# vivek87799/lightweight-human-pose-estimation.pytorch

Hardware: AMD Instinct MI355X
Metric: frames/sec end-to-end (net+grouping) at 368px (higher is better)
Workload: dtype f32; 1 GPU; batch=1 per GPU, 368x656 frames, 1 refinement stage(s), fp32 convs / f32+f64 post, resident normalised NCHW input -> key-points + pose entries on host; 3 frame batch(es) in flight per GPU (3 engine stream(s), each step a complete pass); global_batch=1, parallelism=dp1 (frames sharded, no data-path collective), 3 stream(s) per GPU

## Files before the change

lightweight-human-pose-estimation.pytorch_amd/csrc/lwp_internal.h:

```cpp
#pragma once
#include <hip/hip_runtime.h>
#include <stdint.h>
#include <algorithm>
#include <cstdio>
#include <string>
#include <vector>

#include "../../include/lwpose.h"

namespace lwp {

struct ParamSpec {
    std::string key;
    int64_t shape[4];
    int ndim;
    int role;
};
std::vector<ParamSpec> param_table(int nref, int C, int NH, int NP);

enum LayerKind { L_STEM = 0, L_DW = 1, L_GEMM = 2, L_DWPW = 3 };
enum Act { ACT_NONE = 0, ACT_RELU = 1, ACT_ELU = 2 };
enum KClass { KC_STEM = 0, KC_DW = 1, KC_PW = 2, KC_C3 = 3, KC_POST = 4, KC_OTHER = 5, KC_COUNT = 6 };

struct BufRef {
    int buf = -1;
    int coff = 0;
    int ld = 0;
};

struct WBlock {
    std::string conv_key;
    int out_off, in_off, cout, cin;
};

struct Layer {
    int kind = L_GEMM;
    std::string name;
    std::string conv_key;
    std::string bn_key;
    bool has_bias = false;
    int cin = 0, cout = 0, ks = 1, stride = 1, dil = 1, act = ACT_NONE;
    BufRef src, dst, res;
    int out_index = -1;
    int out_index2 = -1, out_split = 0;
    std::vector<WBlock> blocks;
    int64_t macs_per_pixel = 0;
    int fuse = LWP_MARK_NONE;
    size_t w_off = 0, b_off = 0;
    int cin_pad = 0, cout_pad = 0;
    std::string conv2_key, bn2_key;
    int act2 = ACT_NONE;
    size_t w2_off = 0, b2_off = 0;
};

struct BufSpec {
    int level;
    int channels;
    bool has_pad = false;
};

struct Graph {
    int nref, C, NH, NP;
    std::vector<BufSpec> bufs;
    std::vector<Layer> layers;
    size_t blob_floats = 0;
    int cat_buf = -1;
    int cat_channels = 0;
    int dtype = LWP_F32;
};
Graph build_graph(int nref, int C, int NH, int NP, bool fuse_dwpw, int dtype, bool merge_heads = true);

struct TrainPlan {
    std::vector<Layer> layers;
    std::vector<BufSpec> bufs;
    std::vector<int> cats;
    int cpm_conv = -1;
    int cpm_in = -1;
    int cut = -1;
    std::vector<int> dw_copy, nores_copy;
    enum { GRAD_ALWAYS = 0, GRAD_NEVER = 1, GRAD_ON_DEMAND = 2 };
    std::vector<char> grad_mode;
};
TrainPlan build_train_plan(const Graph& g, int scope = LWP_TRAIN_STAGES);
uint16_t f32_to_f16_rne(float f);
uint16_t f32_to_bf16_rne(float f);

struct HostTensor {
    const void* ptr;
    int64_t shape[4];
    int ndim;
};
std::string pack_weights(const Graph& g, const std::vector<std::string>& names,
                         const std::vector<HostTensor>& tensors, std::vector<float>& blob);

struct Tuning {
    int stem_ty = 0, stem_wl = -1, stem_debug = 0;
    int dw_tiled = -1, dw_cc = 0, dw_ph = 0;
    int gemm_wp = -1;
    bool has_c3 = false, has_pw = false; int c3[3] = {0, 0, 0}, pw[3] = {0, 0, 0};
    int dwpw_bm = 0, dwpw_nw = 0, dwpw_debug = 0, dwpwh_debug = 0;
    int dwpw_pipe = -1;
    int dwpw_tiled_wgs = 0;
    int dwpw_tiled = -1;
    int dwpw_pp_grid = 0;
    int dwpw_pp = -1;
    int heads_rm = 0;
    int gemmh_fold = -1;
    int gemmh_persist = -1, gemmh_ar_off = 0, gemmh_ar_force = 0, gemmh_debug = 0;
    bool has_gemmh_ar = false, has_gemmh = false; int gemmh_ar[4] = {0, 0, 0, 0}, gemmh[4] = {0, 0, 0, 0};
    int upsample_tiled = -1;
    int max_frames_per_pass = 0;
    int peak_tile = -1, pair_form = -1;
    int dwpw_lds_pad_kb = 0;
    int host_fetch_dma = -1;
    int ms_tx = 0;
    int ms_vec = -1;
    int ms_fused = -1;
    int heads_f32_lds = -1;
    int post_nchw = -1;
    int heads_f32_max_m = 0;
    int fuse_dwpw = -1, merge_heads = -1, fuse_heads = -1;
    int pre_batch_vec = -1;
    int post_stream = -1, post_generic = -1;
};
Tuning tuning_from_env();
const Tuning& default_tuning();
constexpr int kVariantCap = 64;
#define LWP_VARIANT(p, ...) do { if ((p).variant) snprintf((p).variant, lwp::kVariantCap, __VA_ARGS__); } while (0)

struct StemParams {
    const float* __restrict__ in;
    const float* __restrict__ w;
    const float* __restrict__ bias;
    float* __restrict__ out;
    int N, H, W, Ho, Wo;
    int f16 = 0;
    const float* zeros = nullptr;
    const Tuning* tune = nullptr; char* variant = nullptr;
};
struct DwParams {
    const float* in; int in_ld;
    const float* w;
    const float* bias;
    float* out; int out_ld;
    int N, Hi, Wi, Ho, Wo, C, stride, dil, act;
    const Tuning* tune = nullptr; char* variant = nullptr;
};
struct GemmParams {
    const float* in; int in_ld;
    int f16 = 0;
    const float* w;
    const float* wf = nullptr;
    const float* bias;
    float* out; int out_ld;
    const float* res; int res_ld;
    float* out_nchw;
    float* out_nchw2 = nullptr;
    int out_split = 0;
    const float* zeros;
    int N, H, W, cin_pad, cout, cout_pad, ks, dil, act;
    int debug = 0;
    const Tuning* tune = nullptr; char* variant = nullptr;
    const void* w2 = nullptr; const float* bias2 = nullptr; void* out2 = nullptr; int out2_ld = 0, act2 = 0;
    bool* fused2 = nullptr;
};
struct DwPwParams {
    const float* in; int in_ld;
    int f16 = 0;
    const float* dw_w;
    const float* pw_w;
    const float* pw_b;
    float* out; int out_ld;
    const float* res; int res_ld;
    const float* zeros;
    int N, Hi, Wi, Ho, Wo, C, cout, stride, dil, act_dw, act_pw;
    int debug = 0;
    const Tuning* tune = nullptr; char* variant = nullptr;
};
bool dwpw_supported(int C, int cout);
hipError_t launch_dwpw(const DwPwParams& p, hipStream_t s);
hipError_t try_dwpw_tiled_f32(const DwPwParams& p, hipStream_t s, bool* used);
// ... 386 lines not shown
```

lightweight-human-pose-estimation.pytorch_amd/csrc/net_kernels.hip:

```cpp
#include <cstdio>
#include <cstdlib>

#include <type_traits>
#include "lwp_internal.h"

namespace lwp {

typedef float f32x4 __attribute__((ext_vector_type(4)));
typedef float f32x2 __attribute__((ext_vector_type(2)));
typedef float f32x16 __attribute__((ext_vector_type(16)));

__device__ __forceinline__ float elu_negative(float v) {
    const float p = v * (1.f + v * (0.5f + v * (1.f / 6.f + v * (1.f / 24.f + v * (1.f / 120.f + v * (1.f / 720.f + v * (1.f / 5040.f)))))));
    return v > -0.5f ? p : __expf(v) - 1.0f;
}
__device__ __forceinline__ float apply_act(float v, int act) {
    if (act == ACT_RELU) return fmaxf(v, 0.0f);
    if (act == ACT_ELU) return v > 0.0f ? v : elu_negative(v);
    return v;
}

constexpr int ST_TX = 32;
template <bool BF16, int ST_TY, int PY = 1, int DBG = 0, bool WL = false, bool F16 = false>
__global__ void __launch_bounds__(ST_TY * ST_TX) stem_kernel(StemParams p) {
// ... 635 lines not shown
                acc = __builtin_amdgcn_mfma_f32_32x32x2f32(av[s].z, bv[s].z, acc, 0, 0, 0);
                acc = __builtin_amdgcn_mfma_f32_32x32x2f32(av[s].w, bv[s].w, acc, 0, 0, 0);
            }
        }
        if (nxt < nsteps) {
            store_step();
#pragma unroll
            for (int s = 0; s < BK / 8; ++s) bv[s] = b_nxt[s];
        }
    }

    float resv[16];
    const bool has_res = p.res != nullptr && g == 0 && n < p.cout;
    if (has_res) {
#pragma unroll
        for (int i = 0; i < 16; ++i) {
            const int m = m0 + (i & 3) + 8 * (i >> 2) + 4 * h;
            resv[i] = m < M ? p.res[(int64_t)m * p.res_ld + n] : 0.f;
        }
    }
    if (KS > 1) {
        __syncthreads();
        float* red = smem;
        if (g > 0) {
#pragma unroll
            for (int i = 0; i < 16; ++i) red[(((g - 1) * WN + wn) * 16 + i) * 64 + lane] = acc[i];
        }
        __syncthreads();
        if (g > 0) return;
#pragma unroll 1
        for (int gg = 1; gg < KS; ++gg)
#pragma unroll
            for (int i = 0; i < 16; ++i) acc[i] += red[(((gg - 1) * WN + wn) * 16 + i) * 64 + lane];
    }

    if (n < p.cout) {
        const int HW = p.H * p.W;
#pragma unroll
        for (int i = 0; i < 16; ++i) {
            const int m = m0 + (i & 3) + 8 * (i >> 2) + 4 * h;
            if (m < M) {
                float v = apply_act(acc[i] + bias, p.act);
                if (has_res) v += resv[i];
                p.out[(int64_t)m * p.out_ld + n] = v;
                if (p.out_nchw || p.out_nchw2) {
                    const int img = m / HW, pix = m - img * HW;
                    const int c0 = p.out_split > 0 ? p.out_split : p.cout;
                    if (n < c0) { if (p.out_nchw) p.out_nchw[((int64_t)img * c0 + n) * HW + pix] = v; }
                    else if (p.out_nchw2) p.out_nchw2[((int64_t)img * (p.cout - c0) + (n - c0)) * HW + pix] = v;
                }
            }
        }
    }
}

template <int BN, int KS, int KSZ>
static hipError_t launch_gemm_wp_k(const GemmParams& p, hipStream_t s) {
    const int64_t M = (int64_t)p.N * p.H * p.W;
    if (M >= (1ll << 31) - 64) return hipErrorInvalidValue;
    const int64_t tiles = ((M + 31) / 32) * (p.cout_pad / BN);
    constexpr int NWV = (BN / 32) * KS;
    size_t lds = (size_t)NWV * 32 * LDS_LD * sizeof(float);
    const size_t red = (size_t)(KS - 1) * (BN / 32) * 16 * 64 * sizeof(float);
    if (red > lds) lds = red;
    if (!p.wf) return hipErrorInvalidValue;
    static LdsAttrOnce attr;
    if (lds > 64 * 1024) {
        hipError_t e = attr.ensure((const void*)gemm_wp_kernel<BN, KS, KSZ>, (int)lds);
        if (e != hipSuccess) return e;
    }
    hipLaunchKernelGGL((gemm_wp_kernel<BN, KS, KSZ>), dim3((unsigned)tiles), dim3(NWV * 64), lds, s, p);
    return hipGetLastError();
}
template <int BN, int KS>
static hipError_t launch_gemm_wp_t(const GemmParams& p, hipStream_t s) {
    if (p.ks == 3) return launch_gemm_wp_k<BN, KS, 3>(p, s);
    if (p.ks == 1) return launch_gemm_wp_k<BN, KS, 1>(p, s);
    return hipErrorInvalidValue;
}

#ifndef AR_PF
#define AR_PF 2
#endif
template <int BN, int KS, int KSZ>
__global__ void __launch_bounds__((BN / 32) * KS * 64) gemm_ar_kernel(GemmParams p) {
    constexpr int WN = BN / 32;
    constexpr int GT = WN * 64;
    extern __shared__ __attribute__((aligned(16))) float smem[];
    const int tid = threadIdx.x, lane = tid & 63;
    const int wave = __builtin_amdgcn_readfirstlane(tid >> 6);
    const int g = wave / WN, wn = wave % WN;
    const int r = lane & 31, h = lane >> 5;

    const int M = p.N * p.H * p.W;
    const int ntn = p.cout_pad / BN;
    int bid = blockIdx.x;
    {
        const int nwg = gridDim.x, q = nwg >> 3, rem = nwg & 7, xcd = bid & 7;
        bid = (xcd < rem ? xcd * (q + 1) : rem * (q + 1) + (xcd - rem) * q) + (bid >> 3);
    }
    const int tile_m = bid / ntn, tile_n = bid % ntn;
    const int m0 = tile_m * 32;
    const int n0 = tile_n * BN + wn * 32;
    const int n = n0 + r;
    const float bias = n < p.cout ? p.bias[n] : 0.f;

    const int kpt = p.cin_pad / BK;
    const int nb = g < kpt ? (kpt - g + KS - 1) / KS : 0;
    const int nb_max = (kpt + KS - 1) / KS;
    const int seg = KSZ == 3 ? 32 + 2 * p.dil : 32;
    const int R = KSZ == 3 ? 3 * seg : 32;
    float* Ag = smem + (size_t)g * (nb_max * R + 1) * LDS_LD;
    float* zrow = Ag + (size_t)nb_max * R * LDS_LD;

    const __amdgpu_buffer_rsrc_t arsrc = __builtin_amdgcn_make_buffer_rsrc((void*)p.in, 0, (int)((int64_t)M * p.in_ld * 4), 0x00020000);
    {
        const int t = tid - g * GT;
        const int col = (t & 7) * 4;
        const int total = nb * R;
        for (int base = 0; base < total; base += 8 * (GT / 8)) {
            f32x4 tmp[8];
#pragma unroll
            for (int u = 0; u < 8; ++u) {
                const int ch = base + (t >> 3) + u * (GT / 8);
                const int chc = ch < total ? ch : 0;
                const int j = chc / R, row = chc - j * R;
                int64_t idx;
                if (KSZ == 3) {
                    const int sd = row / seg, rw = row - sd * seg;
                    idx = (int64_t)m0 + (int64_t)(sd - 1) * p.dil * p.W - p.dil + rw;
                } else {
                    idx = (int64_t)m0 + row;
                }
                const bool ok = ch < total && idx >= 0 && idx < M;
                tmp[u] = __builtin_bit_cast(f32x4, __builtin_amdgcn_raw_buffer_load_b128(arsrc, ok ? (unsigned)(((int)idx * p.in_ld + (g + j * KS) * BK + col) * 4) : 0x80000000u, 0, 0));
            }
#pragma unroll
            for (int u = 0; u < 8; ++u) {
                const int ch = base + (t >> 3) + u * (GT / 8);
                if (ch < total) *(f32x4*)(Ag + (size_t)ch * LDS_LD + col) = tmp[u];
            }
        }
        if (t < 9) *(f32x4*)(zrow + 4 * t) = f32x4{0.f, 0.f, 0.f, 0.f};
    }

    const int mrow = m0 + r;
    const bool row_ok = mrow < M;
    const int mm = row_ok ? mrow : 0;
    const int qy = mm / p.W;
    const int x = mm - qy * p.W, y = qy % p.H;
    unsigned valid = 0;
#pragma unroll
    for (int t = 0; t < KSZ * KSZ; ++t) {
        const int yy = y + (KSZ == 3 ? (t / 3 - 1) * p.dil : 0), xx = x + (KSZ == 3 ? (t % 3 - 1) * p.dil : 0);
        if (row_ok && yy >= 0 && yy < p.H && xx >= 0 && xx < p.W) valid |= 1u << t;
    }
    constexpr int taps = KSZ * KSZ;
    const int my_steps = nb * taps;
    const __amdgpu_buffer_rsrc_t wrsrc = __builtin_amdgcn_make_buffer_rsrc((void*)p.wf, 0, 0x7fffffff, 0x00020000);
    const unsigned b_tile = (unsigned)__builtin_amdgcn_readfirstlane(n0 >> 5) * 4096u;
    const unsigned b_step = (unsigned)(p.cout_pad >> 5) * 4096u;
    auto load_b = [&](int i, f32x4* dst) {
        const int j = i / taps, tap = i - j * taps;
        const unsigned soff = (unsigned)(tap * kpt + g + j * KS) * b_step + b_tile;
#pragma unroll
        for (int s = 0; s < BK / 8; ++s) dst[s] = __builtin_bit_cast(f32x4, __builtin_amdgcn_raw_buffer_load_b128(wrsrc, lane * 16 + s * 1024, soff, 0));
    };
    constexpr int PF = AR_PF;
    f32x4 bv[PF][BK / 8];
    if (my_steps > 0) {
#pragma unroll
        for (int u = 0; u < PF - 1; ++u) load_b(u < my_steps ? u : my_steps - 1, bv[u]);
    }
    __syncthreads();

    f32x16 acc = {0.f, 0.f, 0.f, 0.f, 0.f, 0.f, 0.f, 0.f, 0.f, 0.f, 0.f, 0.f, 0.f, 0.f, 0.f, 0.f};
    const float* a_lane = Ag + (size_t)r * LDS_LD + 4 * h;
    const float* z_lane = zrow + 4 * h;
    auto one = [&](int i, auto P_) {
        constexpr int P = decltype(P_)::value;
        const int nxt = i + PF - 1 < my_steps ? i + PF - 1 : my_steps - 1;
        load_b(nxt, bv[(P + PF - 1) % PF]);
        const int j = i / taps, tap = i - j * taps;
        int roff = j * R;
        if (KSZ == 3) roff += (tap / 3) * seg + (tap % 3) * p.dil;
        const float* a = (valid >> tap) & 1u ? a_lane + (size_t)roff * LDS_LD : z_lane;
        f32x4 av[BK / 8];
#pragma unroll
        for (int s = 0; s < BK / 8; ++s) av[s] = *(const f32x4*)(a + 8 * s);
#pragma unroll
        for (int s = 0; s < BK / 8; ++s) {
            acc = __builtin_amdgcn_mfma_f32_32x32x2f32(av[s].x, bv[P][s].x, acc, 0, 0, 0);
            acc = __builtin_amdgcn_mfma_f32_32x32x2f32(av[s].y, bv[P][s].y, acc, 0, 0, 0);
            acc = __builtin_amdgcn_mfma_f32_32x32x2f32(av[s].z, bv[P][s].z, acc, 0, 0, 0);
            acc = __builtin_amdgcn_mfma_f32_32x32x2f32(av[s].w, bv[P][s].w, acc, 0, 0, 0);
        }
    };
    int i = 0;
    for (; i + PF <= my_steps; i += PF) {
        one(i, std::integral_constant<int, 0>{});
        if (PF > 1) one(i + 1, std::integral_constant<int, 1 % PF>{});
        if (PF > 2) one(i + 2, std::integral_constant<int, 2 % PF>{});
        if (PF > 3) one(i + 3, std::integral_constant<int, 3 % PF>{});
    }
    if (i < my_steps) { one(i, std::integral_constant<int, 0>{}); ++i; }
    if (PF > 2 && i < my_steps) { one(i, std::integral_constant<int, 1 % PF>{}); ++i; }
    if (PF > 3 && i < my_steps) { one(i, std::integral_constant<int, 2 % PF>{}); ++i; }

    constexpr int EPG = 16 / KS;
    const int e0 = g * EPG;
    float resv[EPG];
    const bool has_res = p.res != nullptr && n < p.cout;
    if (has_res) {
#pragma unroll
        for (int u = 0; u < EPG; ++u) {
            const int e = e0 + u;
            const int m = m0 + (e & 3) + 8 * (e >> 2) + 4 * h;
            resv[u] = m < M ? p.res[(int64_t)m * p.res_ld + n] : 0.f;
        }
    }
    float outv[EPG];
    if (KS > 1) {
        __syncthreads();
        float* red = smem;
#pragma unroll
        for (int e = 0; e < 16; ++e) red[((g * WN + wn) * 16 + e) * 64 + lane] = acc[e];
        __syncthreads();
#pragma unroll
        for (int u = 0; u < EPG; ++u) {
            float v = red[((0 * WN + wn) * 16 + e0 + u) * 64 + lane];
#pragma unroll
            for (int gg = 1; gg < KS; ++gg) v += red[((gg * WN + wn) * 16 + e0 + u) * 64 + lane];
            outv[u] = v;
        }
    } else {
#pragma unroll
        for (int u = 0; u < EPG; ++u) outv[u] = acc[u];
    }

    if (n < p.cout) {
        const int HW = p.H * p.W;
#pragma unroll
        for (int u = 0; u < EPG; ++u) {
            const int e = e0 + u;
            const int m = m0 + (e & 3) + 8 * (e >> 2) + 4 * h;
            if (m < M) {
                float v = apply_act(outv[u] + bias, p.act);
                if (has_res) v += resv[u];
                p.out[(int64_t)m * p.out_ld + n] = v;
                if (p.out_nchw || p.out_nchw2) {
                    const int img = m / HW, pix = m - img * HW;
                    const int c0 = p.out_split > 0 ? p.out_split : p.cout;
                    if (n < c0) { if (p.out_nchw) p.out_nchw[((int64_t)img * c0 + n) * HW + pix] = v; }
                    else if (p.out_nchw2) p.out_nchw2[((int64_t)img * (p.cout - c0) + (n - c0)) * HW + pix] = v;
                }
            }
        }
    }
}

template <int BN, int KS, int KSZ>
static hipError_t launch_gemm_ar_k(const GemmParams& p, hipStream_t s, bool* fits) {
    const int64_t M = (int64_t)p.N * p.H * p.W;
    *fits = false;
    if (M >= (1ll << 31) - 64 || !p.wf) return hipSuccess;
    if (M * p.in_ld * 4 >= (1ll << 31)) return hipSuccess;
    const int kpt = p.cin_pad / BK, nb_max = (kpt + KS - 1) / KS;
    const int R = KSZ == 3 ? 3 * (32 + 2 * p.dil) : 32;
    size_t lds = (size_t)KS * ((size_t)nb_max * R + 1) * LDS_LD * sizeof(float);
    const size_t red = (size_t)KS * (BN / 32) * 16 * 64 * sizeof(float);
    if (red > lds) lds = red;
    if (lds > 150 * 1024) return hipSuccess;
    *fits = true;
    constexpr int NWV = (BN / 32) * KS;
    const int64_t tiles = ((M + 31) / 32) * (p.cout_pad / BN);
    static LdsAttrOnce attr;
    {
        hipError_t e = attr.ensure((const void*)gemm_ar_kernel<BN, KS, KSZ>, 150 * 1024);
        if (e != hipSuccess) return e;
    }
    hipLaunchKernelGGL((gemm_ar_kernel<BN, KS, KSZ>), dim3((unsigned)tiles), dim3(NWV * 64), lds, s, p);
    return hipGetLastError();
}
template <int BN, int KS>
static hipError_t launch_gemm_ar_t(const GemmParams& p, hipStream_t s, bool* fits) {
    if (p.ks == 3) return launch_gemm_ar_k<BN, KS, 3>(p, s, fits);
    if (p.ks == 1) return launch_gemm_ar_k<BN, KS, 1>(p, s, fits);
    *fits = false;
    return hipSuccess;
}

struct GemmCfg { int bm, bn, ks; };

static hipError_t dispatch_gemm(const GemmParams& p, hipStream_t s, GemmCfg c) {
    const Tuning& T = p.tune ? *p.tune : default_tuning();
    const bool wp_set = T.gemm_wp >= 0;
    if (c.bm == 32 && !wp_set) {
        bool fits = false;
        hipError_t e = hipSuccess;
#define AR_CASE(BN_, KS_) if (c.bn == BN_ && c.ks == KS_) e = launch_gemm_ar_t<BN_, KS_>(p, s, &fits);
        AR_CASE(64, 1) AR_CASE(64, 2) AR_CASE(64, 4) AR_CASE(32, 4) AR_CASE(32, 8)
#undef AR_CASE
        if (fits) LWP_VARIANT(p, "gemm_ar<%d,%d,%d>", c.bn, c.ks, p.ks);
        if (e != hipSuccess || fits) return e;
    }
    if (c.bm == 32 && T.gemm_wp != 0) {
        LWP_VARIANT(p, "gemm_wp<%d,%d,%d>", c.bn, c.ks, p.ks);
#define WP_CASE(BN_, KS_) if (c.bn == BN_ && c.ks == KS_) return launch_gemm_wp_t<BN_, KS_>(p, s);
        WP_CASE(64, 1) WP_CASE(64, 2) WP_CASE(64, 4) WP_CASE(64, 8) WP_CASE(32, 4) WP_CASE(32, 8)
#undef WP_CASE
    }
    LWP_VARIANT(p, "gemm<%d,%d,%d,%d>", c.bm, c.bn, c.ks, p.ks);
#define GEMM_CASE(BM_, BN_, KS_) \
    if (c.bm == BM_ && c.bn == BN_ && c.ks == KS_) return launch_gemm_t<BM_, BN_, KS_>(p, s);
    GEMM_CASE(32, 64, 1) GEMM_CASE(32, 64, 2) GEMM_CASE(32, 64, 4)
    GEMM_CASE(64, 64, 1) GEMM_CASE(64, 64, 2) GEMM_CASE(64, 64, 4)
    GEMM_CASE(64, 128, 1) GEMM_CASE(64, 128, 2)
    GEMM_CASE(128, 128, 1)
    GEMM_CASE(32, 32, 4) GEMM_CASE(32, 32, 8)
#undef GEMM_CASE
    return hipErrorInvalidValue;
}

hipError_t launch_gemm(const GemmParams& p, hipStream_t s) {
    const int64_t M = (int64_t)p.N * p.H * p.W;
    const int nsteps = p.ks * p.ks * (p.cin_pad / BK);
    GemmCfg c{64, 64, 1};
    const Tuning& T = p.tune ? *p.tune : default_tuning();
    if (p.ks == 3 ? T.has_c3 : T.has_pw) {
        const int* v = p.ks == 3 ? T.c3 : T.pw;
        const GemmCfg o{v[0], v[1], v[2]};
        if (o.bn > 0 && (p.cout_pad % o.bn) == 0) return dispatch_gemm(p, s, o);
    }
    const int64_t t64 = ((M + 63) / 64) * (p.cout_pad / 64);
    const int64_t t32 = ((M + 31) / 32) * (p.cout_pad / 64);
    const int64_t t128 = (p.cout_pad % 128 == 0) ? ((M + 127) / 128) * (p.cout_pad / 128) : 0;
    const int64_t rounds128 = (t128 + 511) / 512;
    if (t128 >= 400 && (t128 >= 2048 || t128 * 5 >= rounds128 * 512 * 4)) {
        c = GemmCfg{128, 128, 1};
    } else if (t64 >= 400) {
        c = GemmCfg{64, 64, (t64 < 1024 && nsteps >= 8) ? 2 : 1};
    } else if (p.cout_pad == 64 && nsteps >= 16) {
        c = GemmCfg{32, 32, 8};
    } else {
        c = GemmCfg{32, 64, nsteps >= 4 ? 4 : (nsteps >= 2 ? 2 : 1)};
        if (t32 >= 1024 && c.ks > 2) c.ks = 2;
    }
    return dispatch_gemm(p, s, c);
}

constexpr int DWPW_F32_APAD = 4;
template <int BM, int NW, int DBG = 0, int ACT = -1>
__global__ void __launch_bounds__(NW * 64) dwpw_kernel(DwPwParams p) {
    const int act_dw = ACT >= 0 ? ACT : p.act_dw, act_pw = ACT >= 0 ? ACT : p.act_pw;
    constexpr int NT = NW * 64;
    constexpr int RT = BM / 16;
    extern __shared__ __attribute__((aligned(16))) float dsm[];
    const int ldA = p.C + DWPW_F32_APAD;
    float* At = dsm;

    const int tid = threadIdx.x, lane = tid & 63;
    const int wave = blockIdx.y * NW + (tid >> 6);
    const int wave_u = __builtin_amdgcn_readfirstlane(wave);
    const __amdgpu_buffer_rsrc_t wrsrc = __builtin_amdgcn_make_buffer_rsrc((void*)p.pw_w, 0, 0x7fffffff, 0x00020000);
    const int nwt = gridDim.y * NW;
// ... 48 lines not shown
        for (; grp < BM / PXG; grp += gadv) {
            const int row0 = grp * PXG;
            if (p.stride == 1 && p.dil == 1 && m + PXG <= M32 && xo + PXG <= Wo) {
                const int base = ((img * p.Hi + yo) * p.Wi + xo) * pix_b + c * 4;
                f32x4 win[3][PXG + 2];
#pragma unroll
                for (int ky = 0; ky < 3; ++ky) {
                    const int yy = yo + ky - 1;
                    const bool rok = yy >= 0 && yy < p.Hi;
#pragma unroll
                    for (int j = 0; j < PXG + 2; ++j) {
                        const int xx = xo + j - 1;
                        win[ky][j] = ldw((rok && xx >= 0 && xx < p.Wi) ? (unsigned)(base + (ky - 1) * row_b + (j - 1) * pix_b) : 0x80000000u);
                    }
                }
#pragma unroll
                for (int i = 0; i < PXG; ++i) {
                    f32x4 acc = bias;
#pragma unroll
                    for (int t = 0; t < 9; ++t) acc += win[t / 3][i + t % 3] * wv[t];
                    acc.x = apply_act(acc.x, act_dw); acc.y = apply_act(acc.y, act_dw);
                    acc.z = apply_act(acc.z, act_dw); acc.w = apply_act(acc.w, act_dw);
                    *(f32x4*)(At + (row0 + i) * ldA + c) = acc;
                }
            } else {
                int xi = xo, yi = yo, im = img;
#pragma unroll
                for (int i = 0; i < PXG; ++i) {
                    const bool ok = m + i < M32;
                    const int yc = yi * p.stride, xc = xi * p.stride;
                    const int base = ((im * p.Hi + yc) * p.Wi + xc) * pix_b + c * 4;
                    f32x4 x[9];
#pragma unroll
                    for (int t = 0; t < 9; ++t) {
                        const int dy = (t / 3 - 1) * p.dil, dx = (t % 3 - 1) * p.dil;
                        const bool in = ok && yc + dy >= 0 && yc + dy < p.Hi && xc + dx >= 0 && xc + dx < p.Wi;
                        x[t] = ldw(in ? (unsigned)(base + dy * row_b + dx * pix_b) : 0x80000000u);
                    }
                    f32x4 acc = bias;
#pragma unroll
                    for (int t = 0; t < 9; ++t) acc += x[t] * wv[t];
                    acc.x = apply_act(acc.x, act_dw); acc.y = apply_act(acc.y, act_dw);
                    acc.z = apply_act(acc.z, act_dw); acc.w = apply_act(acc.w, act_dw);
                    *(f32x4*)(At + (row0 + i) * ldA + c) = acc;
                    if (++xi == Wo) { xi = 0; if (++yi == Ho) { yi = 0; ++im; } }
                }
            }
            m += adv;
            xo += adv_x; yo += adv_y;
            if (xo >= Wo) { xo -= Wo; ++yo; }
            while (yo >= Ho) { yo -= Ho; ++img; }
        }
    }
    __syncthreads();

    f32x4 acc[RT][2];
#pragma unroll
    for (int a = 0; a < RT; ++a) { acc[a][0] = f32x4{0.f, 0.f, 0.f, 0.f}; acc[a][1] = f32x4{0.f, 0.f, 0.f, 0.f}; }
    const float* a_lane = At + r16 * ldA + 4 * q;
    auto one = [&](int step, auto P_) {
        constexpr int P = decltype(P_)::value;
        const int nxt = step + PF - 1 < nsteps ? step + PF - 1 : nsteps - 1;
        if (!(DBG & 2)) load_b(nxt, bw[(P + PF - 1) % PF]);
        __builtin_amdgcn_sched_barrier(0);
        if (DBG & 4) return;
        const f32x4* bcur = bw[P];
#pragma unroll
        for (int u = 0; u < 2; ++u) {
            f32x4 av[RT];
#pragma unroll
            for (int a = 0; a < RT; ++a) av[a] = *(const f32x4*)(a_lane + a * 16 * ldA + step * 32 + 16 * u);
#pragma unroll
            for (int j = 0; j < 4; ++j) {
#pragma unroll
                for (int t = 0; t < 2; ++t) {
                    const int v = u * 8 + j * 2 + t;
                    const float b = bcur[v >> 2][v & 3];
#pragma unroll
                    for (int a = 0; a < RT; ++a) acc[a][t] = __builtin_amdgcn_mfma_f32_16x16x4f32(b, av[a][j], acc[a][t], 0, 0, 0);
                }
            }
        }
    };
    int s0 = 0;
    for (; s0 + PF <= nsteps; s0 += PF) {
        one(s0, std::integral_constant<int, 0>{});
        if (PF > 1) one(s0 + 1, std::integral_constant<int, 1 % PF>{});
        if (PF > 2) one(s0 + 2, std::integral_constant<int, 2 % PF>{});
    }
    if (s0 < nsteps) { one(s0, std::integral_constant<int, 0>{}); ++s0; }
    if (PF > 2 && s0 < nsteps) { one(s0, std::integral_constant<int, 1 % PF>{}); ++s0; }
#pragma unroll
    for (int t = 0; t < 2; ++t) {
        const int n = wave * 32 + t * 16 + 4 * q;
        const f32x4 bias = *(const f32x4*)(p.pw_b + n);
#pragma unroll
        for (int a = 0; a < RT; ++a) {
            const int64_t m = m0 + a * 16 + r16;
            if (m < M) {
                f32x4 v = acc[a][t] + bias;
                v.x = apply_act(v.x, act_pw); v.y = apply_act(v.y, act_pw);
                v.z = apply_act(v.z, act_pw); v.w = apply_act(v.w, act_pw);
                if (p.res) v += *(const f32x4*)(p.res + m * p.res_ld + n);
                *(f32x4*)(p.out + m * p.out_ld + n) = v;
            }
        }
    }
}

template <int BM, int NW, int DBG = 0, int ACT = -1>
static hipError_t launch_dwpw_t(const DwPwParams& p, hipStream_t s) {
    const int64_t M = (int64_t)p.N * p.Ho * p.Wo;
    const size_t lds = (size_t)BM * (p.C + DWPW_F32_APAD) * sizeof(float);
    if ((int64_t)p.N * p.Hi * p.Wi * p.in_ld * 4 >= (1ll << 31)) return hipErrorInvalidValue;
    const int nsplit = (p.cout / 32) / NW;
    static LdsAttrOnce attr;
    if (lds > 48 * 1024) {
        hipError_t e = attr.ensure((const void*)dwpw_kernel<BM, NW, DBG, ACT>, 160 * 1024);
        if (e != hipSuccess) return e;
    }
    hipLaunchKernelGGL((dwpw_kernel<BM, NW, DBG, ACT>), dim3((unsigned)((M + BM - 1) / BM), nsplit), dim3(NW * 64), lds, s, p);
    return hipGetLastError();
}

template <int C>
__global__ void __launch_bounds__(1024) dwpw_pipe_kernel(DwPwParams p, int ntiles) {
    constexpr int BM = 32, NT = 1024, RT = BM / 16, NSTEP = C / 32;
    constexpr int ldA = C + DWPW_F32_APAD;
    constexpr int CG = C / 4;
    constexpr int PAR = NT / CG;
    constexpr int NIT = BM / PAR;
    static_assert(NIT * 4 == NSTEP, "one pixel per four K steps");
    extern __shared__ __attribute__((aligned(16))) float dsm[];
    float* Wd = dsm + 2 * BM * ldA;
    const int tid = threadIdx.x, lane = tid & 63;
    const int wave_u = __builtin_amdgcn_readfirstlane(tid >> 6);
    const int r16 = lane & 15, q = lane >> 4;
    const int M32 = p.N * p.Ho * p.Wo;
    const int G = gridDim.x;
    int bid = blockIdx.x;
    {
        const int qq = G >> 3, rem = G & 7, xcd = bid & 7;
        bid = (xcd < rem ? xcd * (qq + 1) : rem * (qq + 1) + (xcd - rem) * qq) + (bid >> 3);
    }
    for (int i = tid * 4; i < 10 * C; i += NT * 4) *(f32x4*)(Wd + i) = *(const f32x4*)(p.dw_w + i);
    const __amdgpu_buffer_rsrc_t wrsrc = __builtin_amdgcn_make_buffer_rsrc((void*)p.pw_w, 0, 0x7fffffff, 0x00020000);
    const __amdgpu_buffer_rsrc_t irsrc = __builtin_amdgcn_make_buffer_rsrc((void*)p.in, 0, (int)((int64_t)p.N * p.Hi * p.Wi * p.in_ld * 4), 0x00020000);
    const int pix_b = p.in_ld * 4, row_b = p.Wi * pix_b;
    const int c = (tid % CG) * 4, prow = tid / CG;
    constexpr int NU = 16;
    f32x4 bw[2][4];
    auto load_b = [&](int step, f32x4* dst) {
        const unsigned soff = (unsigned)(step * NU + wave_u) * 4096u;
#pragma unroll
        for (int j = 0; j < 4; ++j) dst[j] = __builtin_bit_cast(f32x4, __builtin_amdgcn_raw_buffer_load_b128(wrsrc, lane * 16 + j * 1024, soff, 0));
    };
    f32x4 win[9], pacc;
    auto p_piece = [&](int tl, int it, int j, float* Adst) {
        if (j == 0) {
            const int m = tl * BM + it * PAR + prow;
            const bool ok = m < M32;
            const unsigned q1 = (unsigned)m / (unsigned)p.Wo;
            const int xo = m - (int)q1 * p.Wo;
            const int img = (int)(q1 / (unsigned)p.Ho);
            const int yo = (int)q1 - img * p.Ho;
            const int yc = yo * p.stride, xc = xo * p.stride;
            const int base = ((img * p.Hi + yc) * p.Wi + xc) * pix_b + c * 4;
#pragma unroll
            for (int t = 0; t < 9; ++t) {
                const int dy = (t / 3 - 1) * p.dil, dx = (t % 3 - 1) * p.dil;
                const bool in = ok && yc + dy >= 0 && yc + dy < p.Hi && xc + dx >= 0 && xc + dx < p.Wi;
                win[t] = __builtin_bit_cast(f32x4, __builtin_amdgcn_raw_buffer_load_b128(irsrc, in ? (unsigned)(base + dy * row_b + dx * pix_b) : 0x80000000u, 0, 0));
            }
        } else if (j == 1) {
            pacc = *(const f32x4*)(Wd + 9 * C + c);
#pragma unroll
            for (int t = 0; t < 4; ++t) pacc += win[t] * *(const f32x4*)(Wd + t * C + c);
        } else if (j == 2) {
#pragma unroll
            for (int t = 4; t < 9; ++t) pacc += win[t] * *(const f32x4*)(Wd + t * C + c);
        } else {
            f32x4 v = pacc;
            v.x = fmaxf(v.x, 0.f); v.y = fmaxf(v.y, 0.f); v.z = fmaxf(v.z, 0.f); v.w = fmaxf(v.w, 0.f);
            *(f32x4*)(Adst + (it * PAR + prow) * ldA + c) = v;
        }
    };
// ... 383 lines not shown
    for (int i = 0; i < PT; ++i) {
        if (!mok[i]) continue;
        const int m = mr[i];
        const int img = m / HW, pix = m - img * HW;
#pragma unroll
        for (int t = 0; t < 4; ++t) {
            const int n = 16 * t + 4 * q;
            if (n >= p.cout) continue;
            f32x4 v = acc2[i][t];
            v += *(const f32x4*)(p.b1 + n);
            if (out_vec && n + 3 < p.cout) *(f32x4*)(out + (int64_t)m * p.out_ld + n) = v;
            else {
#pragma unroll
                for (int r = 0; r < 4; ++r) if (n + r < p.cout) out[(int64_t)m * p.out_ld + n + r] = v[r];
            }
            if (p.out_nchw || p.out_nchw2) {
#pragma unroll
                for (int r = 0; r < 4; ++r) {
                    const int ch = n + r;
                    if (ch >= p.cout) continue;
                    if (ch < c0) { if (p.out_nchw) p.out_nchw[((int64_t)img * c0 + ch) * HW + pix] = v[r]; }
                    else if (p.out_nchw2) p.out_nchw2[((int64_t)img * (p.cout - c0) + (ch - c0)) * HW + pix] = v[r];
                }
            }
        }
    }
}

bool heads_f32_supported(int cin_pad, int hidden, int cout_pad, int64_t M, const Tuning* tune) {
    const int64_t max_m = (tune && tune->heads_f32_max_m > 0) ? tune->heads_f32_max_m : 4096;
    if (!(cin_pad == 128 && hidden % 16 == 0 && hidden >= 128 && hidden <= 4096 && cout_pad == 64)) return false;
    if (M <= max_m) return true;
    return hidden % HL_HC == 0 && !(tune && tune->heads_f32_lds == 0);
}

hipError_t launch_heads_f32(const HeadsParams& p, hipStream_t s) {
    constexpr int NW = 8;
    const int64_t M = (int64_t)p.N * p.H * p.W;
    if (M * p.in_ld * 4 >= (1ll << 31) || (p.in_ld & 3)) return hipErrorInvalidValue;
    const int64_t max_m = (p.tune && p.tune->heads_f32_max_m > 0) ? p.tune->heads_f32_max_m : 4096;
    if (M > max_m) {
        constexpr int PT = 2;
        if (M >= (1ll << 31) - 64 * PT) return hipErrorInvalidValue;
        const size_t lds2 = (size_t)(2 * HL_HC * HL_LD0 + 2 * 64 * HL_LD1 + p.hidden) * sizeof(float);
        static LdsAttrOnce attr;
        hipError_t e = attr.ensure((const void*)heads_f32_lds_kernel<PT>, 96 * 1024);
        if (e != hipSuccess) return e;
        LWP_VARIANT(p, "heads_f32_lds<%d>", PT);
        hipLaunchKernelGGL(heads_f32_lds_kernel<PT>, dim3((unsigned)((M + 64 * PT - 1) / (64 * PT))), dim3(256), lds2, s, p);
        return hipGetLastError();
    }
    const size_t lds = (size_t)NW * 2 * 4 * 64 * 4 * sizeof(float);
    const unsigned nheads = p.out_split > 0 ? 2u : 1u;
    if (p.out_split < 0 || p.out_split >= p.cout || (nheads == 2 && p.hidden % 32)) return hipErrorInvalidValue;
    static LdsAttrOnce attr8;
    hipError_t e = attr8.ensure((const void*)heads_f32_kernel<NW>, 64 * 1024);
    if (e != hipSuccess) return e;
    LWP_VARIANT(p, "heads_f32<%d>", NW);
    hipLaunchKernelGGL(heads_f32_kernel<NW>, dim3((unsigned)((M + 31) / 32) * nheads), dim3(NW * 64), lds, s, p);
    return hipGetLastError();
}

const Tuning& default_tuning() { static const Tuning t; return t; }
Tuning tuning_from_env() {
    Tuning t;
    auto geti = [](const char* name, int* dst) { const char* e = getenv(name); if (e && e[0]) *dst = atoi(e); };
    auto digit = [](const char* name, int* dst) { const char* e = getenv(name); if (e && e[0]) *dst = e[0] - '0'; };
    geti("LWP_STEM_TY", &t.stem_ty); digit("LWP_STEM_WL", &t.stem_wl); geti("LWP_STEM_DEBUG", &t.stem_debug);
    digit("LWP_DW_TILED", &t.dw_tiled); geti("LWP_DW_CC", &t.dw_cc); geti("LWP_DW_PH", &t.dw_ph);
    digit("LWP_GEMM_WP", &t.gemm_wp);
    if (const char* e = getenv("LWP_GEMM_C3")) t.has_c3 = sscanf(e, "%d,%d,%d", &t.c3[0], &t.c3[1], &t.c3[2]) == 3;
    if (const char* e = getenv("LWP_GEMM_PW")) t.has_pw = sscanf(e, "%d,%d,%d", &t.pw[0], &t.pw[1], &t.pw[2]) == 3;
    geti("LWP_DWPW_BM", &t.dwpw_bm); geti("LWP_DWPW_NW", &t.dwpw_nw); geti("LWP_DWPW_DEBUG", &t.dwpw_debug); geti("LWP_DWPWH_DEBUG", &t.dwpwh_debug);
    digit("LWP_DWPW_PIPE", &t.dwpw_pipe);
    digit("LWP_DWPW_TILED", &t.dwpw_tiled); geti("LWP_DWPW_TILED_WGS", &t.dwpw_tiled_wgs);
    digit("LWP_DWPW_PP", &t.dwpw_pp); geti("LWP_DWPW_PP_GRID", &t.dwpw_pp_grid);
    geti("LWP_HEADS_RM", &t.heads_rm);
    digit("LWP_GEMMH_PERSIST", &t.gemmh_persist); digit("LWP_GEMMH_FOLD", &t.gemmh_fold);
    if (const char* e = getenv("LWP_GEMMH_AR")) {
        if (e[0] == '0' && e[1] == 0) t.gemmh_ar_off = 1;
        else t.has_gemmh_ar = sscanf(e, "%d,%d,%d,%d", &t.gemmh_ar[0], &t.gemmh_ar[1], &t.gemmh_ar[2], &t.gemmh_ar[3]) == 4;
    }
    if (const char* e = getenv("LWP_GEMMH_AR_FORCE")) t.gemmh_ar_force = e[0] == '1';
    geti("LWP_GEMMH_DEBUG", &t.gemmh_debug);
    if (const char* e = getenv("LWP_GEMMH")) t.has_gemmh = sscanf(e, "%d,%d,%d,%d", &t.gemmh[0], &t.gemmh[1], &t.gemmh[2], &t.gemmh[3]) == 4;
    digit("LWP_UPSAMPLE_TILED", &t.upsample_tiled);
    digit("LWP_PEAK_TILE", &t.peak_tile); digit("LWP_PAIR_FORM", &t.pair_form); digit("LWP_POST_NCHW", &t.post_nchw); digit("LWP_HEADS_F32_LDS", &t.heads_f32_lds); digit("LWP_MS_FUSED", &t.ms_fused); digit("LWP_MS_VEC", &t.ms_vec); geti("LWP_MS_TX", &t.ms_tx); digit("LWP_HOST_FETCH_DMA", &t.host_fetch_dma); geti("LWP_DWPW_LDS_PAD", &t.dwpw_lds_pad_kb);
    geti("LWP_HEADS_F32_MAXM", &t.heads_f32_max_m);
    geti("LWP_MAX_FRAMES_PER_PASS", &t.max_frames_per_pass);
    digit("LWP_FUSE_DWPW", &t.fuse_dwpw); digit("LWP_MERGE_HEADS", &t.merge_heads); digit("LWP_FUSE_HEADS", &t.fuse_heads);
    digit("LWP_PRE_BATCH_VEC", &t.pre_batch_vec); digit("LWP_POST_STREAM", &t.post_stream); digit("LWP_POST_GENERIC", &t.post_generic);
    return t;
}

__global__ void __launch_bounds__(256) nchw_from_nhwc_kernel(const float* src, int src_ld, float* dst, int N, int HW, int C) {
    const int64_t total = (int64_t)N * C * HW;
    const int64_t idx = (int64_t)blockIdx.x * blockDim.x + threadIdx.x;
    if (idx >= total) return;
    const int pix = (int)(idx % HW);
    const int64_t t = idx / HW;
    const int c = (int)(t % C);
    const int n = (int)(t / C);
    dst[idx] = src[((int64_t)n * HW + pix) * src_ld + c];
}
hipError_t launch_nchw_from_nhwc(const float* src, int src_ld, float* dst, int N, int HW, int C, hipStream_t s) {
    const int64_t total = (int64_t)N * C * HW;
    hipLaunchKernelGGL(nchw_from_nhwc_kernel, dim3((unsigned)((total + 255) / 256)), dim3(256), 0, s, src, src_ld, dst, N, HW, C);
    return hipGetLastError();
}

}
```

Measured before the change: 2568 frames/s.

## Specialize gemm_ar by dilation, overlap A/B prologue loads, buffer-load epilogue

Templates the activation-resident GEMM kernel on compile-time dilation, adding a single-round A-tile prologue with precomputed offsets for the common one-block case. The first B prefetch is issued before the validity-mask computation and the LDS stores, so more global loads are in flight at once. The epilogue switches to buffer loads and stores with out-of-bounds offsets instead of branches, and the fused dw+pw kernel hoists its bias and residual loads ahead of the store loop. This adds more template instantiations and ablation debug variants behind a compile flag, plus new 2GB range checks.

```diff
diff --git a/lightweight-human-pose-estimation.pytorch_amd/csrc/lwp_internal.h b/lightweight-human-pose-estimation.pytorch_amd/csrc/lwp_internal.h
--- a/lightweight-human-pose-estimation.pytorch_amd/csrc/lwp_internal.h
+++ b/lightweight-human-pose-estimation.pytorch_amd/csrc/lwp_internal.h
@@ -97,6 +97,7 @@
     int stem_ty = 0, stem_wl = -1, stem_debug = 0;
     int dw_tiled = -1, dw_cc = 0, dw_ph = 0;
     int gemm_wp = -1;
+    int gemm_debug = 0;
     bool has_c3 = false, has_pw = false; int c3[3] = {0, 0, 0}, pw[3] = {0, 0, 0};
     int dwpw_bm = 0, dwpw_nw = 0, dwpw_debug = 0, dwpwh_debug = 0;
     int dwpw_pipe = -1;
diff --git a/lightweight-human-pose-estimation.pytorch_amd/csrc/net_kernels.hip b/lightweight-human-pose-estimation.pytorch_amd/csrc/net_kernels.hip
--- a/lightweight-human-pose-estimation.pytorch_amd/csrc/net_kernels.hip
+++ b/lightweight-human-pose-estimation.pytorch_amd/csrc/net_kernels.hip
@@ -741,10 +741,12 @@
 #ifndef AR_PF
 #define AR_PF 2
 #endif
-template <int BN, int KS, int KSZ>
+template <int BN, int KS, int DIL, int DBG, int KSZ>
 __global__ void __launch_bounds__((BN / 32) * KS * 64) gemm_ar_kernel(GemmParams p) {
     constexpr int WN = BN / 32;
     constexpr int GT = WN * 64;
+    constexpr int RPT = GT / 8;
+    constexpr unsigned OOB = 0x80000000u;
     extern __shared__ __attribute__((aligned(16))) float smem[];
     const int tid = threadIdx.x, lane = tid & 63;
     const int wave = __builtin_amdgcn_readfirstlane(tid >> 6);
@@ -758,68 +760,60 @@
         const int nwg = gridDim.x, q = nwg >> 3, rem = nwg & 7, xcd = bid & 7;
         bid = (xcd < rem ? xcd * (q + 1) : rem * (q + 1) + (xcd - rem) * q) + (bid >> 3);
     }
-    const int tile_m = bid / ntn, tile_n = bid % ntn;
+    int tile_m;
+    if ((ntn & (ntn - 1)) == 0) tile_m = bid >> __builtin_ctz(ntn); else tile_m = bid / ntn;
+    const int tile_n = bid - tile_m * ntn;
     const int m0 = tile_m * 32;
     const int n0 = tile_n * BN + wn * 32;
     const int n = n0 + r;
-    const float bias = n < p.cout ? p.bias[n] : 0.f;
 
     const int kpt = p.cin_pad / BK;
     const int nb = g < kpt ? (kpt - g + KS - 1) / KS : 0;
     const int nb_max = (kpt + KS - 1) / KS;
-    const int seg = KSZ == 3 ? 32 + 2 * p.dil : 32;
+    const int dil = KSZ == 3 ? (DIL > 0 ? DIL : p.dil) : 0;
+    const int seg = KSZ == 3 ? 32 + 2 * dil : 32;
     const int R = KSZ == 3 ? 3 * seg : 32;
     float* Ag = smem + (size_t)g * (nb_max * R + 1) * LDS_LD;
     float* zrow = Ag + (size_t)nb_max * R * LDS_LD;
 
     const __amdgpu_buffer_rsrc_t arsrc = __builtin_amdgcn_make_buffer_rsrc((void*)p.in, 0, (int)((int64_t)M * p.in_ld * 4), 0x00020000);
-    {
-        const int t = tid - g * GT;
-        const int col = (t & 7) * 4;
-        const int total = nb * R;
-        for (int base = 0; base < total; base += 8 * (GT / 8)) {
-            f32x4 tmp[8];
-#pragma unroll
-            for (int u = 0; u < 8; ++u) {
-                const int ch = base + (t >> 3) + u * (GT / 8);
-                const int chc = ch < total ? ch : 0;
-                const int j = chc / R, row = chc - j * R;
-                int64_t idx;
-                if (KSZ == 3) {
-                    const int sd = row / seg, rw = row - sd * seg;
-                    idx = (int64_t)m0 + (int64_t)(sd - 1) * p.dil * p.W - p.dil + rw;
-                } else {
-                    idx = (int64_t)m0 + row;
-                }
-                const bool ok = ch < total && idx >= 0 && idx < M;
-                tmp[u] = __builtin_bit_cast(f32x4, __builtin_amdgcn_raw_buffer_load_b128(arsrc, ok ? (unsigned)(((int)idx * p.in_ld + (g + j * KS) * BK + col) * 4) : 0x80000000u, 0, 0));
-            }
-#pragma unroll
-            for (int u = 0; u < 8; ++u) {
-                const int ch = base + (t >> 3) + u * (GT / 8);
-                if (ch < total) *(f32x4*)(Ag + (size_t)ch * LDS_LD + col) = tmp[u];
-            }
-        }
-        if (t < 9) *(f32x4*)(zrow + 4 * t) = f32x4{0.f, 0.f, 0.f, 0.f};
-    }
-
-    const int mrow = m0 + r;
-    const bool row_ok = mrow < M;
-    const int mm = row_ok ? mrow : 0;
-    const int qy = mm / p.W;
-    const int x = mm - qy * p.W, y = qy % p.H;
-    unsigned valid = 0;
-#pragma unroll
-    for (int t = 0; t < KSZ * KSZ; ++t) {
-        const int yy = y + (KSZ == 3 ? (t / 3 - 1) * p.dil : 0), xx = x + (KSZ == 3 ? (t % 3 - 1) * p.dil : 0);
-        if (row_ok && yy >= 0 && yy < p.H && xx >= 0 && xx < p.W) valid |= 1u << t;
-    }
+    const int t = tid - g * GT;
+    const int col = (t & 7) * 4, trow = t >> 3;
+    const int total = nb * R;
+    auto a_off = [&](int ch, int j, int row) -> unsigned {
+        int idx = m0 + row;
+        if (KSZ == 3) {
+            const int sd = (row >= seg ? 1 : 0) + (row >= 2 * seg ? 1 : 0);
+            idx = m0 + (sd - 1) * dil * p.W - dil + (row - sd * seg);
+        }
+        const bool ok = ch < total && idx >= 0 && idx < M;
+        return ok ? ((unsigned)idx * (unsigned)p.in_ld + (unsigned)((g + j * KS) * BK + col)) * 4u : OOB;
+    };
+    constexpr int R_CT = KSZ == 1 ? 32 : (DIL > 0 ? 3 * (32 + 2 * DIL) : 0);
+    constexpr int NU1 = R_CT > 0 && (R_CT + RPT - 1) / RPT <= 8 ? (R_CT + RPT - 1) / RPT : 0;
+    const bool one_round = NU1 > 0 && nb == 1;
+    auto a_off1 = [&](int u) -> unsigned {
+        const int row = trow + u * RPT;
+        const int pxb = p.in_ld * 4;
+        int shift = 0;
+        if (KSZ == 3) {
+            const int dw = dil * p.W;
+            shift = row >= 2 * seg ? dw - dil - 2 * seg : (row >= seg ? -dil - seg : -dw - dil);
+        }
+        const int idx = m0 + row + shift;
+        const bool ok = row < R_CT && idx >= 0 && idx < M;
+        const unsigned base = (unsigned)(m0 + trow) * (unsigned)pxb + (unsigned)((g * BK + col) * 4);
+        const int bshift = KSZ == 3 ? (row >= 2 * seg ? (dil * p.W - dil - 2 * seg) * pxb : (row >= seg ? (-dil - seg) * pxb : (-dil * p.W - dil) * pxb)) : 0;
+        return ok ? base + (unsigned)(u * RPT * pxb) + (unsigned)bshift : OOB;
+    };
+
     constexpr int taps = KSZ * KSZ;
     const int my_steps = nb * taps;
     const __amdgpu_buffer_rsrc_t wrsrc = __builtin_amdgcn_make_buffer_rsrc((void*)p.wf, 0, 0x7fffffff, 0x00020000);
     const unsigned b_tile = (unsigned)__builtin_amdgcn_readfirstlane(n0 >> 5) * 4096u;
     const unsigned b_step = (unsigned)(p.cout_pad >> 5) * 4096u;
     auto load_b = [&](int i, f32x4* dst) {
+        if (DBG & 2) return;
         const int j = i / taps, tap = i - j * taps;
         const unsigned soff = (unsigned)(tap * kpt + g + j * KS) * b_step + b_tile;
 #pragma unroll
@@ -827,10 +821,72 @@
     };
     constexpr int PF = AR_PF;
     f32x4 bv[PF][BK / 8];
-    if (my_steps > 0) {
-#pragma unroll
-        for (int u = 0; u < PF - 1; ++u) load_b(u < my_steps ? u : my_steps - 1, bv[u]);
-    }
+    if (DBG & 2) {
+#pragma unroll
+        for (int u = 0; u < PF; ++u)
+#pragma unroll
+            for (int s = 0; s < BK / 8; ++s) bv[u][s] = f32x4{1.f, 1.f, 1.f, 1.f};
+    }
+    unsigned valid = 0;
+    auto prologue = [&](auto ONE_) {
+        constexpr bool ONE = decltype(ONE_)::value;
+        constexpr int NU = ONE ? NU1 : 8;
+        f32x4 tmp[8];
+        auto round = [&](int base) {
+#pragma unroll
+            for (int u = 0; u < 8; ++u) {
+                const int ch = base + trow + u * RPT;
+                const int chc = ch < total ? ch : 0;
+                const int j = chc / R;
+                tmp[u] = __builtin_bit_cast(f32x4, __builtin_amdgcn_raw_buffer_load_b128(arsrc, a_off(ch, j, chc - j * R), 0, 0));
+            }
+        };
+        if (!(DBG & 1)) {
+            if (ONE) {
+#pragma unroll
+                for (int u = 0; u < NU; ++u) tmp[u] = __builtin_bit_cast(f32x4, __builtin_amdgcn_raw_buffer_load_b128(arsrc, a_off1(u), 0, 0));
+            } else if (total > 0) {
+                round(0);
+            }
+        }
+        if (ONE || my_steps > 0) {
+#pragma unroll
+            for (int u = 0; u < PF - 1; ++u) load_b(ONE ? (u < taps ? u : taps - 1) : (u < my_steps ? u : my_steps - 1), bv[u]);
+        }
+        __builtin_amdgcn_sched_barrier(0);
+
+        const int mrow = m0 + r;
+        const bool row_ok = mrow < M;
+        const int mm = row_ok ? mrow : 0;
+        const int qy = mm / p.W;
+        const int x = mm - qy * p.W, y = qy % p.H;
+#pragma unroll
+        for (int tp = 0; tp < KSZ * KSZ; ++tp) {
+            const int yy = y + (KSZ == 3 ? (tp / 3 - 1) * dil : 0), xx = x + (KSZ == 3 ? (tp % 3 - 1) * dil : 0);
+            if (row_ok && yy >= 0 && yy < p.H && xx >= 0 && xx < p.W) valid |= 1u << tp;
+        }
+
+        if (!(DBG & 1)) {
+            if (ONE) {
+#pragma unroll
+                for (int u = 0; u < NU; ++u) {
+                    const int row = trow + u * RPT;
+                    if (row < R_CT) *(f32x4*)(Ag + (size_t)row * LDS_LD + col) = tmp[u];
+                }
+            } else {
+                for (int base = 0; base < total; base += 8 * RPT) {
+                    if (base > 0) round(base);
+#pragma unroll
+                    for (int u = 0; u < 8; ++u) {
+                        const int ch = base + trow + u * RPT;
+                        if (ch < total) *(f32x4*)(Ag + (size_t)ch * LDS_LD + col) = tmp[u];
+                    }
+                }
+            }
+        }
+    };
+    if (one_round) prologue(std::true_type{}); else prologue(std::false_type{});
+    if (t < 9) *(f32x4*)(zrow + 4 * t) = f32x4{0.f, 0.f, 0.f, 0.f};
     __syncthreads();
 
     f32x16 acc = {0.f, 0.f, 0.f, 0.f, 0.f, 0.f, 0.f, 0.f, 0.f, 0.f, 0.f, 0.f, 0.f, 0.f, 0.f, 0.f};
@@ -842,17 +898,21 @@
         load_b(nxt, bv[(P + PF - 1) % PF]);
         const int j = i / taps, tap = i - j * taps;
         int roff = j * R;
-        if (KSZ == 3) roff += (tap / 3) * seg + (tap % 3) * p.dil;
+        if (KSZ == 3) roff += (tap / 3) * seg + (tap % 3) * dil;
         const float* a = (valid >> tap) & 1u ? a_lane + (size_t)roff * LDS_LD : z_lane;
         f32x4 av[BK / 8];
 #pragma unroll
         for (int s = 0; s < BK / 8; ++s) av[s] = *(const f32x4*)(a + 8 * s);
 #pragma unroll
-        for (int s = 0; s < BK / 8; ++s) {
+        for (int s = 0; s < ((DBG & 4) ? 0 : BK / 8); ++s) {
             acc = __builtin_amdgcn_mfma_f32_32x32x2f32(av[s].x, bv[P][s].x, acc, 0, 0, 0);
             acc = __builtin_amdgcn_mfma_f32_32x32x2f32(av[s].y, bv[P][s].y, acc, 0, 0, 0);
             acc = __builtin_amdgcn_mfma_f32_32x32x2f32(av[s].z, bv[P][s].z, acc, 0, 0, 0);
             acc = __builtin_amdgcn_mfma_f32_32x32x2f32(av[s].w, bv[P][s].w, acc, 0, 0, 0);
+        }
+        if (DBG & 4) {
+#pragma unroll
+            for (int s = 0; s < BK / 8; ++s) asm volatile("" :: "v"(av[s]), "v"(bv[P][s]));
         }
     };
     int i = 0;
@@ -865,17 +925,37 @@
     if (i < my_steps) { one(i, std::integral_constant<int, 0>{}); ++i; }
     if (PF > 2 && i < my_steps) { one(i, std::integral_constant<int, 1 % PF>{}); ++i; }
     if (PF > 3 && i < my_steps) { one(i, std::integral_constant<int, 2 % PF>{}); ++i; }
+    if (DBG & 8) {
+        if (p.debug == 0x7fffffff) {
+#pragma unroll
+            for (int e = 0; e < 16; ++e) p.out[e * 64 + lane] = acc[e];
+        }
+        return;
+    }
 
     constexpr int EPG = 16 / KS;
     const int e0 = g * EPG;
+    const bool n_ok = n < p.cout;
+    const __amdgpu_buffer_rsrc_t brsrc = __builtin_amdgcn_make_buffer_rsrc((void*)p.bias, 0, p.cout * 4, 0x00020000);
+    const float bias = __builtin_bit_cast(float, __builtin_amdgcn_raw_buffer_load_b32(brsrc, n_ok ? (unsigned)n * 4u : OOB, 0, 0));
+    unsigned o_off[EPG];
+    bool m_ok[EPG];
+#pragma unroll
+    for (int u = 0; u < EPG; ++u) {
+        const int e = e0 + u;
+        const int m = m0 + (e & 3) + 8 * (e >> 2) + 4 * h;
+        m_ok[u] = m < M && n_ok;
+        o_off[u] = m_ok[u] ? ((unsigned)m * (unsigned)p.out_ld + (unsigned)n) * 4u : OOB;
+    }
     float resv[EPG];
-    const bool has_res = p.res != nullptr && n < p.cout;
+    const bool has_res = p.res != nullptr;
     if (has_res) {
+        const __amdgpu_buffer_rsrc_t rrsrc = __builtin_amdgcn_make_buffer_rsrc((void*)p.res, 0, ((M - 1) * p.res_ld + p.cout) * 4, 0x00020000);
 #pragma unroll
         for (int u = 0; u < EPG; ++u) {
             const int e = e0 + u;
             const int m = m0 + (e & 3) + 8 * (e >> 2) + 4 * h;
-            resv[u] = m < M ? p.res[(int64_t)m * p.res_ld + n] : 0.f;
+            resv[u] = __builtin_bit_cast(float, __builtin_amdgcn_raw_buffer_load_b32(rrsrc, m_ok[u] ? ((unsigned)m * (unsigned)p.res_ld + (unsigned)n) * 4u : OOB, 0, 0));
         }
     }
     float outv[EPG];
@@ -897,33 +977,46 @@
         for (int u = 0; u < EPG; ++u) outv[u] = acc[u];
     }
 
-    if (n < p.cout) {
+    float v[EPG];
+#pragma unroll
+    for (int u = 0; u < EPG; ++u) {
+        v[u] = apply_act(outv[u] + bias, p.act);
+        if (has_res) v[u] += resv[u];
+    }
+    const __amdgpu_buffer_rsrc_t orsrc = __builtin_amdgcn_make_buffer_rsrc((void*)p.out, 0, ((M - 1) * p.out_ld + p.cout) * 4, 0x00020000);
+#pragma unroll
+    for (int u = 0; u < EPG; ++u) __builtin_amdgcn_raw_buffer_store_b32(__builtin_bit_cast(unsigned, v[u]), orsrc, o_off[u], 0, 0);
+    if (p.out_nchw || p.out_nchw2) {
         const int HW = p.H * p.W;
+        const int c0 = p.out_split > 0 ? p.out_split : p.cout;
 #pragma unroll
         for (int u = 0; u < EPG; ++u) {
+            if (!m_ok[u]) continue;
             const int e = e0 + u;
             const int m = m0 + (e & 3) + 8 * (e >> 2) + 4 * h;
-            if (m < M) {
-                float v = apply_act(outv[u] + bias, p.act);
-                if (has_res) v += resv[u];
-                p.out[(int64_t)m * p.out_ld + n] = v;
-                if (p.out_nchw || p.out_nchw2) {
-                    const int img = m / HW, pix = m - img * HW;
-                    const int c0 = p.out_split > 0 ? p.out_split : p.cout;
-                    if (n < c0) { if (p.out_nchw) p.out_nchw[((int64_t)img * c0 + n) * HW + pix] = v; }
-                    else if (p.out_nchw2) p.out_nchw2[((int64_t)img * (p.cout - c0) + (n - c0)) * HW + pix] = v;
-                }
-            }
-        }
-    }
-}
-
+            const int img = m / HW, pix = m - img * HW;
+            if (n < c0) { if (p.out_nchw) p.out_nchw[((int64_t)img * c0 + n) * HW + pix] = v[u]; }
+            else if (p.out_nchw2) p.out_nchw2[((int64_t)img * (p.cout - c0) + (n - c0)) * HW + pix] = v[u];
+        }
+    }
+}
+
+template <int BN, int KS, int DIL, int DBG, int KSZ>
+static hipError_t launch_gemm_ar_i(const GemmParams& p, hipStream_t s, unsigned tiles, size_t lds) {
+    static LdsAttrOnce attr;
+    hipError_t e = attr.ensure((const void*)gemm_ar_kernel<BN, KS, DIL, DBG, KSZ>, 150 * 1024);
+    if (e != hipSuccess) return e;
+    hipLaunchKernelGGL((gemm_ar_kernel<BN, KS, DIL, DBG, KSZ>), dim3(tiles), dim3((BN / 32) * KS * 64), lds, s, p);
+    return hipGetLastError();
+}
 template <int BN, int KS, int KSZ>
 static hipError_t launch_gemm_ar_k(const GemmParams& p, hipStream_t s, bool* fits) {
     const int64_t M = (int64_t)p.N * p.H * p.W;
     *fits = false;
     if (M >= (1ll << 31) - 64 || !p.wf) return hipSuccess;
     if (M * p.in_ld * 4 >= (1ll << 31)) return hipSuccess;
+    if (((M - 1) * p.out_ld + p.cout) * 4 >= (1ll << 31)) return hipSuccess;
+    if (p.res && ((M - 1) * p.res_ld + p.cout) * 4 >= (1ll << 31)) return hipSuccess;
     const int kpt = p.cin_pad / BK, nb_max = (kpt + KS - 1) / KS;
     const int R = KSZ == 3 ? 3 * (32 + 2 * p.dil) : 32;
     size_t lds = (size_t)KS * ((size_t)nb_max * R + 1) * LDS_LD * sizeof(float);
@@ -931,15 +1024,22 @@
     if (red > lds) lds = red;
     if (lds > 150 * 1024) return hipSuccess;
     *fits = true;
-    constexpr int NWV = (BN / 32) * KS;
-    const int64_t tiles = ((M + 31) / 32) * (p.cout_pad / BN);
-    static LdsAttrOnce attr;
-    {
-        hipError_t e = attr.ensure((const void*)gemm_ar_kernel<BN, KS, KSZ>, 150 * 1024);
-        if (e != hipSuccess) return e;
-    }
-    hipLaunchKernelGGL((gemm_ar_kernel<BN, KS, KSZ>), dim3((unsigned)tiles), dim3(NWV * 64), lds, s, p);
-    return hipGetLastError();
+    const unsigned tiles = (unsigned)(((M + 31) / 32) * (p.cout_pad / BN));
+    const int dil = KSZ == 3 && (p.dil == 1 || p.dil == 2) ? p.dil : 0;
+#ifdef LWP_ABLATION
+    const int d = (p.tune ? *p.tune : default_tuning()).gemm_debug;
+    if (BN == 64 && KS == 4 && d) {
+#define AR_DBG(D_) if (d == D_) { \
+            if (KSZ == 1) return launch_gemm_ar_i<64, 4, 0, D_, 1>(p, s, tiles, lds); \
+            if (dil == 1) return launch_gemm_ar_i<64, 4, 1, D_, 3>(p, s, tiles, lds); \
+            if (dil == 2) return launch_gemm_ar_i<64, 4, 2, D_, 3>(p, s, tiles, lds); }
+        AR_DBG(1) AR_DBG(2) AR_DBG(4) AR_DBG(8) AR_DBG(7) AR_DBG(14) AR_DBG(15)
+#undef AR_DBG
+    }
+#endif
+    if (dil == 1) return launch_gemm_ar_i<BN, KS, KSZ == 3 ? 1 : 0, 0, KSZ>(p, s, tiles, lds);
+    if (dil == 2) return launch_gemm_ar_i<BN, KS, KSZ == 3 ? 2 : 0, 0, KSZ>(p, s, tiles, lds);
+    return launch_gemm_ar_i<BN, KS, 0, 0, KSZ>(p, s, tiles, lds);
 }
 template <int BN, int KS>
 static hipError_t launch_gemm_ar_t(const GemmParams& p, hipStream_t s, bool* fits) {
@@ -1154,6 +1254,9 @@
             }
         }
     };
+    f32x4 bias[2];
+#pragma unroll
+    for (int t = 0; t < 2; ++t) bias[t] = *(const f32x4*)(p.pw_b + wave * 32 + t * 16 + 4 * q);
     int s0 = 0;
     for (; s0 + PF <= nsteps; s0 += PF) {
         one(s0, std::integral_constant<int, 0>{});
@@ -1162,18 +1265,27 @@
     }
     if (s0 < nsteps) { one(s0, std::integral_constant<int, 0>{}); ++s0; }
     if (PF > 2 && s0 < nsteps) { one(s0, std::integral_constant<int, 1 % PF>{}); ++s0; }
+    f32x4 resv[RT][2];
+    if (p.res) {
+#pragma unroll
+        for (int t = 0; t < 2; ++t)
+#pragma unroll
+            for (int a = 0; a < RT; ++a) {
+                const int64_t m = m0 + a * 16 + r16;
+                resv[a][t] = m < M ? *(const f32x4*)(p.res + m * p.res_ld + wave * 32 + t * 16 + 4 * q) : f32x4{0.f, 0.f, 0.f, 0.f};
+            }
+    }
 #pragma unroll
     for (int t = 0; t < 2; ++t) {
         const int n = wave * 32 + t * 16 + 4 * q;
-        const f32x4 bias = *(const f32x4*)(p.pw_b + n);
 #pragma unroll
         for (int a = 0; a < RT; ++a) {
             const int64_t m = m0 + a * 16 + r16;
             if (m < M) {
-                f32x4 v = acc[a][t] + bias;
+                f32x4 v = acc[a][t] + bias[t];
                 v.x = apply_act(v.x, act_pw); v.y = apply_act(v.y, act_pw);
                 v.z = apply_act(v.z, act_pw); v.w = apply_act(v.w, act_pw);
-                if (p.res) v += *(const f32x4*)(p.res + m * p.res_ld + n);
+                if (p.res) v += resv[a][t];
                 *(f32x4*)(p.out + m * p.out_ld + n) = v;
             }
         }
@@ -1723,7 +1835,7 @@
         else t.has_gemmh_ar = sscanf(e, "%d,%d,%d,%d", &t.gemmh_ar[0], &t.gemmh_ar[1], &t.gemmh_ar[2], &t.gemmh_ar[3]) == 4;
     }
     if (const char* e = getenv("LWP_GEMMH_AR_FORCE")) t.gemmh_ar_force = e[0] == '1';
-    geti("LWP_GEMMH_DEBUG", &t.gemmh_debug);
+    geti("LWP_GEMMH_DEBUG", &t.gemmh_debug); geti("LWP_GEMM_DEBUG", &t.gemm_debug);
     if (const char* e = getenv("LWP_GEMMH")) t.has_gemmh = sscanf(e, "%d,%d,%d,%d", &t.gemmh[0], &t.gemmh[1], &t.gemmh[2], &t.gemmh[3]) == 4;
     digit("LWP_UPSAMPLE_TILED", &t.upsample_tiled);
     digit("LWP_PEAK_TILE", &t.peak_tile); digit("LWP_PAIR_FORM", &t.pair_form); digit("LWP_POST_NCHW", &t.post_nchw); digit("LWP_HEADS_F32_LDS", &t.heads_f32_lds); digit("LWP_MS_FUSED", &t.ms_fused); digit("LWP_MS_VEC", &t.ms_vec); geti("LWP_MS_TX", &t.ms_tx); digit("LWP_HOST_FETCH_DMA", &t.host_fetch_dma); geti("LWP_DWPW_LDS_PAD", &t.dwpw_lds_pad_kb);
```

Result: faster. 2711 frames/s (median of 6 runs) (+5.6%).
